# felipefelixarias/a2cat-vn-pytorch

Hardware: NVIDIA B200
Metric: env-steps/s (obs gather+step+reset) (higher is better)
Workload: dtype u8

## Files before the change

a2cat-vn-pytorch_b200/csrc/vn_common.cuh:

```cuda
#pragma once
#include <cuda_runtime.h>
#include <stdint.h>

#include <cstdarg>
#include <cstdio>

#include "vn_b200.h"

#if defined(__CUDA_ARCH__) && (__CUDA_ARCH__ < 1000)
#error "libvn_b200 is written for sm_100a (B200) only"
#endif

namespace vn {

void set_error(const char *fmt, ...);
int32_t launch_result(const char *what, cudaError_t e);
template <typename... P>
inline bool aligned16(const P *...p) {
    return ((reinterpret_cast<uintptr_t>(p) | ... | uintptr_t(0)) & 15) == 0;
}
int sm_count();
int32_t ensure_smem(const void *kernel, int bytes);
template <typename... KArgs>
int32_t ensure_smem(void (*kernel)(KArgs...), int bytes) {
// ... 123 lines not shown
__device__ __forceinline__ uint64_t l2_policy_evict_last() {
    uint64_t p;
    asm volatile("createpolicy.fractional.L2::evict_last.b64 %0, 1.0;" : "=l"(p));
    return p;
}
__device__ __forceinline__ void bulk_g2s_hint(void *smem_dst, const void *gmem_src, uint32_t bytes, uint64_t *bar,
                                              uint64_t policy) {
    asm volatile(
        "cp.async.bulk.shared::cluster.global.mbarrier::complete_tx::bytes.L2::cache_hint [%0], [%1], %2, [%3], %4;" ::"r"(
            smem_u32(smem_dst)),
        "l"(gmem_src), "r"(bytes), "r"(smem_u32(bar)), "l"(policy)
        : "memory");
}
__device__ __forceinline__ void bulk_s2g_hint(void *gmem_dst, const void *smem_src, uint32_t bytes, uint64_t policy) {
    asm volatile("cp.async.bulk.global.shared::cta.bulk_group.L2::cache_hint [%0], [%1], %2, %3;" ::"l"(gmem_dst),
                 "r"(smem_u32(smem_src)), "r"(bytes), "l"(policy)
                 : "memory");
}
__device__ __forceinline__ void bulk_commit() { asm volatile("cp.async.bulk.commit_group;" ::: "memory"); }
template <int N>
__device__ __forceinline__ void bulk_wait_read() {
    asm volatile("cp.async.bulk.wait_group.read %0;" ::"n"(N) : "memory");
}
__device__ __forceinline__ void fence_proxy_async() { asm volatile("fence.proxy.async.shared::cta;" ::: "memory"); }

}
```

a2cat-vn-pytorch_b200/csrc/vn_env.cu:

```cuda
#include <atomic>
#include <chrono>
#include <cstring>
#include <map>
#include <mutex>
#include <string>
#include <utility>

#include "vn_common.cuh"

namespace vn {

static thread_local std::string g_error;
static unsigned long long *g_gather_trace = nullptr;
static std::atomic<long long> g_launches{0};

void set_error(const char *fmt, ...) {
    char buf[512];
    va_list ap;
    va_start(ap, fmt);
    vsnprintf(buf, sizeof(buf), fmt, ap);
    va_end(ap);
    g_error = buf;
}

// ... 209 lines not shown
__device__ __forceinline__ void add_stats(uint64_t *stats, const EnvStats &s) {
    unsigned long long *st = reinterpret_cast<unsigned long long *>(stats);
    if (s.episodes) {
        atomicAdd(st + VN_STAT_EPISODES, (unsigned long long)s.episodes);
        atomicAdd(reinterpret_cast<double *>(st + VN_STAT_RETURN_SUM), (double)s.ret);
        atomicAdd(st + VN_STAT_LENGTH_SUM, (unsigned long long)s.len);
        if (s.succ) atomicAdd(st + VN_STAT_SUCCESSES, (unsigned long long)s.succ);
        if (s.trunc) atomicAdd(st + VN_STAT_TRUNCATIONS, (unsigned long long)s.trunc);
    }
    if (s.coll) atomicAdd(st + VN_STAT_COLLISIONS, (unsigned long long)s.coll);
    if (s.steps) atomicAdd(st + VN_STAT_STEPS, (unsigned long long)s.steps);
    if (s.resets) atomicAdd(st + VN_STAT_RESETS, (unsigned long long)s.resets);
    if (s.skipped) atomicAdd(st + VN_STAT_ROWS_SKIPPED, (unsigned long long)s.skipped);
}

__device__ __forceinline__ void signal_host(const vn_step_out_t &out) {
    __syncthreads();
    if (threadIdx.x == 0) {
        __threadfence_system();
        *reinterpret_cast<volatile uint32_t *>(out.host_seq + blockIdx.x) = out.seq;
    }
}

template <bool kReset>
__global__ void __launch_bounds__(kStepThreads) vn_step_kernel(const StepParams p) {
    const bool defer_wait = (p.out.flags & VN_STEP_ACTIONS_READY) && !(p.out.flags & VN_STEP_NO_OVERLAP) &&
                            p.out.gather_desc != nullptr;
    if (!defer_wait) asm volatile("griddepcontrol.wait;" ::: "memory");
    asm volatile("griddepcontrol.launch_dependents;" ::: "memory");
    const int i = blockIdx.x * blockDim.x + threadIdx.x;
    if (i == 0 && p.out.sched) p.out.sched[p.out.parity & 1] = 0u;
    EnvStats st;
    if (i < p.env.n_envs) {
        int rec, grec;
        step_env<kReset>(p, i, st, rec, grec);
        if (p.out.gather_desc)
            reinterpret_cast<int2 *>(p.out.gather_desc)[(size_t)(p.out.parity & 1) * p.env.n_envs + i] =
                make_int2(rec, grec);
    }

    if (p.out.stats) {
        const EnvStats w = warp_reduce(st);
        if ((threadIdx.x & 31) == 0) add_stats(p.out.stats, w);
    }
    if (p.out.host_seq) signal_host(p.out);
    if (defer_wait) asm volatile("griddepcontrol.wait;" ::: "memory");
}

struct GatherParams {
    vn_store_t store;
    const int2 *desc;
    const int32_t *obs_state;
    const int32_t *goal;
    const uint8_t *did_reset;
    uint8_t *obs[VN_MAX_PLANES];
    uint8_t *goal_obs[VN_MAX_PLANES];
    unsigned int *sched;
    int32_t n;
    int32_t parity;
    int32_t early_release;
    unsigned long long *trace;
};

__device__ __forceinline__ unsigned long long globaltimer_ns() {
    unsigned long long t;
    asm volatile("mov.u64 %0, %globaltimer;" : "=l"(t));
    return t;
}

template <int kThreads, int kUnroll>
__device__ __forceinline__ void copy_segment16(const uint8_t *__restrict__ src, uint8_t *__restrict__ dst, int n16) {
    const int4 *s = reinterpret_cast<const int4 *>(src);
    int4 *d = reinterpret_cast<int4 *>(dst);
    int base = threadIdx.x;
    for (; base + (kUnroll - 1) * kThreads < n16; base += kUnroll * kThreads) {
        int4 v[kUnroll];
#pragma unroll
        for (int k = 0; k < kUnroll; ++k) v[k] = ld_stream16(s + base + k * kThreads);
#pragma unroll
        for (int k = 0; k < kUnroll; ++k) st_stream16(d + base + k * kThreads, v[k]);
    }
    int4 v[kUnroll];
// ... 26 lines not shown
                if (p.obs[pl])
                    copy_segment16<kThreads, kUnroll>(src + p.store.plane_off[pl],
                                                      p.obs[pl] + (size_t)env * p.store.plane_bytes[pl],
                                                      p.store.plane_bytes[pl] >> 4);
            }
        }
        if (grec >= 0) {
            const uint8_t *gsrc = p.store.base + (size_t)grec * p.store.state_pitch;
#pragma unroll 1
            for (int pl = 0; pl < p.store.n_planes; ++pl) {
                if (p.goal_obs[pl])
                    copy_segment16<kThreads, kUnroll>(gsrc + p.store.plane_off[pl],
                                                      p.goal_obs[pl] + (size_t)env * p.store.plane_bytes[pl],
                                                      p.store.plane_bytes[pl] >> 4);
            }
        }
    }
}

struct L2Policies {
    uint64_t load, store;
};

template <typename F>
__device__ __forceinline__ void bulk_copy_slice(const vn_store_t &st, const uint8_t *src, uint8_t *const *dst, int env,
                                                int slice, int split, uint8_t *smem, uint64_t *bar, uint32_t &parity,
                                                const L2Policies &pol, F while_loading, bool whole) {
    bulk_wait_read<0>();
    int total = 0;
#pragma unroll 1
    for (int pl = 0; pl < st.n_planes; ++pl)
        if (dst[pl]) {
            const int n16 = st.plane_bytes[pl] >> 4, per = (n16 + split - 1) / split;
            const int lo = min(slice * per, n16), hi = min(lo + per, n16);
            total += hi - lo;
        }
    if (total == 0) return;
    if (whole && split == 1) {
        int first = -1, last = -1;
        for (int pl = 0; pl < st.n_planes; ++pl)
            if (dst[pl]) {
                if (first < 0) first = pl;
                last = pl;
            }
        const uint32_t base = (uint32_t)st.plane_off[first];
        const uint32_t span = (uint32_t)st.plane_off[last] + (uint32_t)st.plane_bytes[last] - base;
        mbar_expect_tx(bar, span);
        bulk_g2s_hint(smem, src + base, span, bar, pol.load);
        while_loading();
        mbar_wait(bar, parity & 1u);
        parity ^= 1u;
        for (int pl = first; pl <= last; ++pl)
            if (dst[pl])
                bulk_s2g_hint(dst[pl] + (size_t)env * st.plane_bytes[pl], smem + ((uint32_t)st.plane_off[pl] - base),
                              (uint32_t)st.plane_bytes[pl], pol.store);
        bulk_commit();
        return;
    }
    mbar_expect_tx(bar, (uint32_t)total << 4);
    int off = 0;
#pragma unroll 1
    for (int pl = 0; pl < st.n_planes; ++pl)
        if (dst[pl]) {
            const int n16 = st.plane_bytes[pl] >> 4, per = (n16 + split - 1) / split;
            const int lo = min(slice * per, n16), hi = min(lo + per, n16);
            if (hi > lo)
                bulk_g2s_hint(smem + ((size_t)off << 4), src + st.plane_off[pl] + ((size_t)lo << 4),
                              (uint32_t)(hi - lo) << 4, bar, pol.load);
            off += hi - lo;
        }
    while_loading();
    mbar_wait(bar, parity & 1u);
    parity ^= 1u;
    off = 0;
#pragma unroll 1
    for (int pl = 0; pl < st.n_planes; ++pl)
        if (dst[pl]) {
            const int n16 = st.plane_bytes[pl] >> 4, per = (n16 + split - 1) / split;
            const int lo = min(slice * per, n16), hi = min(lo + per, n16);
            if (hi > lo)
                bulk_s2g_hint(dst[pl] + (size_t)env * st.plane_bytes[pl] + ((size_t)lo << 4), smem + ((size_t)off << 4),
                              (uint32_t)(hi - lo) << 4, pol.store);
            off += hi - lo;
        }
    bulk_commit();
}

__global__ void __launch_bounds__(32) vn_gather_bulk_kernel(const GatherParams p, int split, unsigned int *sched,
                                                            int whole) {
    extern __shared__ __align__(128) uint8_t smem[];
    __shared__ uint64_t bar;
    if (threadIdx.x != 0) return;
    unsigned long long *tr = p.trace ? p.trace + (size_t)blockIdx.x * 16 : nullptr;
    if (tr) {
        tr[0] = globaltimer_ns();
        unsigned int smid;
        asm volatile("mov.u32 %0, %smid;" : "=r"(smid));
        tr[6] = smid;
    }
    mbar_init(&bar, 1);
    asm volatile("fence.mbarrier_init.release.cluster;" ::: "memory");
    asm volatile("griddepcontrol.wait;" ::: "memory");
    if (p.early_release) asm volatile("griddepcontrol.launch_dependents;" ::: "memory");
    if (tr) tr[1] = globaltimer_ns();
    int n_units = 0;
    uint32_t parity = 0;
    const L2Policies pol{l2_policy_evict_last(), l2_policy_evict_first()};
    const int units = p.n * split;
    const bool dynamic = sched != nullptr;
    auto unit_desc = [&](int u) -> int2 {
        if (u >= units) return make_int2(-1, -1);
        const int env = split == 1 ? u : u / split;
        if (p.desc) return p.desc[env];
        int2 d = make_int2(p.obs_state[env], -1);
        if (p.goal && (!p.did_reset || p.did_reset[env])) d.y = p.goal[env];
        return d;
    };
    int u = (int)blockIdx.x;
    int2 d = unit_desc(u);
    while (u < units) {
        const int env = split == 1 ? u : u / split;
        const int slice = split == 1 ? 0 : u - env * split;
        int u_next = 0;
        int2 d_next = make_int2(-1, -1);
        bool have_next = false;
        auto fetch_next = [&]() {
            if (have_next) return;
            u_next = dynamic ? (int)gridDim.x + (int)atomicAdd(sched, 1u) : u + (int)gridDim.x;
            d_next = unit_desc(u_next);
            have_next = true;
        };
        if (d.x >= 0) {
            const uint8_t *src = p.store.base + (size_t)d.x * p.store.state_pitch;
            bulk_copy_slice(p.store, src, p.obs, env, slice, split, smem, &bar, parity, pol, fetch_next,
                            (whole & 1) != 0);
        }
        if (d.y >= 0) {
            const uint8_t *gsrc = p.store.base + (size_t)d.y * p.store.state_pitch;
            bulk_copy_slice(p.store, gsrc, p.goal_obs, env, slice, split, smem, &bar, parity, pol, fetch_next,
                            (whole & 2) != 0);
        }
        fetch_next();
        if (tr) {
            if (n_units == 0) tr[2] = globaltimer_ns();
            tr[3] = globaltimer_ns();
            if (n_units < 8) tr[8 + n_units] = tr[3] | ((unsigned long long)(d.x < 0 && d.y < 0) << 63);
            ++n_units;
        }
        u = u_next;
        d = d_next;
    }
    bulk_wait_read<0>();
    if (tr) {
        tr[4] = globaltimer_ns();
        tr[5] = (unsigned long long)n_units;
    }
}

constexpr int kFusedWarps = 4;
constexpr int kFusedPerSm = 4;

template <bool kReset>
__global__ void __launch_bounds__(kFusedWarps * 32) vn_step_fused_kernel(const StepParams sp, const GatherParams gp) {
    extern __shared__ __align__(128) uint8_t smem[];
    __shared__ uint64_t bar[kFusedWarps];
    __shared__ int s_rec, s_grec;
    const int warp = threadIdx.x >> 5;
    if (threadIdx.x < kFusedWarps) mbar_init(&bar[threadIdx.x], 1);
    asm volatile("fence.mbarrier_init.release.cluster;" ::: "memory");
    asm volatile("griddepcontrol.wait;" ::: "memory");
    asm volatile("griddepcontrol.launch_dependents;" ::: "memory");
    const int env = blockIdx.x;
    if (threadIdx.x == 0) {
        EnvStats st;
        int rec, grec;
        step_env<kReset>(sp, env, st, rec, grec);
        if (sp.out.stats) add_stats(sp.out.stats, st);
        if (sp.out.gather_desc)
// ... 186 lines not shown
}

static int32_t check_rows_aligned(const GatherParams &gp) {
    for (int pl = 0; pl < gp.store.n_planes; ++pl) {
        VN_REQUIRE(aligned16(gp.obs[pl]), "gather: obs[%d] must be 16-byte aligned", pl);
        VN_REQUIRE(aligned16(gp.goal_obs[pl]), "gather: goal_obs[%d] must be 16-byte aligned", pl);
    }
    return VN_OK;
}

static int plane_set_bytes(const vn_store_t &st, uint8_t *const *dst, bool use, int *span, bool *contiguous) {
    int sum = 0, first = -1, last = -1;
    for (int pl = 0; pl < st.n_planes; ++pl)
        if (use && dst[pl]) {
            sum += st.plane_bytes[pl];
            if (first < 0) first = pl;
            last = pl;
        }
    *span = first < 0 ? 0 : st.plane_off[last] + st.plane_bytes[last] - st.plane_off[first];
    *contiguous = first >= 0 && last > first && *span - sum <= 128 * (last - first);
    return sum;
}

static int32_t launch_gather(const GatherParams &gp, int32_t variant, cudaStream_t stream) {
    if (gp.n == 0) return VN_OK;
    int32_t rc = check_rows_aligned(gp);
    if (rc) return rc;
    if (variant == VN_GATHER_AUTO || variant == VN_GATHER_FUSED || variant == VN_GATHER_PERSISTENT)
        variant = VN_GATHER_BULK;
    if (variant == VN_GATHER_LDG) {
        constexpr int kThreads = 256;
        return launch(vn_gather_ldg_kernel<kThreads, 4>, "vn_gather_ldg_kernel", dim3(gp.n), dim3(kThreads), 0, stream,
                      true, gp);
    }
    if (variant != VN_GATHER_BULK) {
        set_error("gather: unknown variant %d", variant);
        return VN_EINVAL;
    }
    int split = gp.n < 2 * sm_count() ? min(16, (2 * sm_count() + gp.n - 1) / gp.n) : 1;
    int per_env = 0, per_goal = 0;
    for (int pl = 0; pl < gp.store.n_planes; ++pl) {
        if (gp.obs[pl]) per_env += gp.store.plane_bytes[pl];
        if (gp.goal && gp.goal_obs[pl]) per_goal += gp.store.plane_bytes[pl];
    }
    split = max(split, (max(per_env, per_goal) + 52 * 1024 - 1) / (52 * 1024));
    int smem_obs = 0, smem_goal = 0;
    for (int pl = 0; pl < gp.store.n_planes; ++pl) {
        const int n16 = gp.store.plane_bytes[pl] >> 4, per = (n16 + split - 1) / split;
        if (gp.obs[pl]) smem_obs += per << 4;
        if (gp.goal && gp.goal_obs[pl]) smem_goal += per << 4;
    }
    int smem = max(smem_obs, smem_goal), whole = 0;
    if (split == 1) {
        int span_o, span_g;
        bool co, cg;
        plane_set_bytes(gp.store, gp.obs, true, &span_o, &co);
        plane_set_bytes(gp.store, gp.goal_obs, gp.goal != nullptr, &span_g, &cg);
        if (co) smem = max(smem, span_o);
        if (cg) smem = max(smem, span_g);
        whole = (co ? 1 : 0) | (cg ? 2 : 0);
    }
    VN_REQUIRE(smem <= 200 * 1024, "gather(bulk): %d bytes of planes per env exceed shared memory", smem);
    rc = ensure_smem(vn_gather_bulk_kernel, smem);
    if (rc) return rc;
    const int grid = (int)min((int64_t)gp.n * split, (int64_t)sm_count() * ctas_per_sm(smem));
    return launch(vn_gather_bulk_kernel, "vn_gather_bulk_kernel", dim3(grid), dim3(32), (size_t)smem, stream, true, gp,
                  split, gp.sched ? gp.sched + (gp.parity & 1) : nullptr, whole);
}
// ... 40 lines not shown
                  dim3(kStepThreads), 0, static_cast<cudaStream_t>(stream), true, sp);
}

static int32_t make_gather_params(GatherParams &gp, const vn_store_t *store, const vn_envs_t *envs,
                                  const vn_step_out_t *out, bool *any) {
    int32_t rc = validate_store(store);
    if (rc) return rc;
    VN_REQUIRE(envs->goal, "envs: null pointer");
    VN_REQUIRE(out && out->obs_state, "out: obs_state is required");
    gp.store = *store;
    gp.obs_state = out->obs_state;
    gp.n = envs->n_envs;
    bool any_goal = false, any_obs = false;
    for (int pl = 0; pl < VN_MAX_PLANES; ++pl) {
        gp.obs[pl] = pl < store->n_planes ? out->obs[pl] : nullptr;
        gp.goal_obs[pl] = pl < store->n_planes ? out->goal_obs[pl] : nullptr;
        any_goal |= gp.goal_obs[pl] != nullptr;
        any_obs |= gp.obs[pl] != nullptr;
    }
    gp.goal = any_goal ? envs->goal : nullptr;
    gp.did_reset = out->did_reset;
    gp.sched = out->sched;
    gp.parity = out->parity;
    gp.early_release = 1;
    gp.trace = g_gather_trace;
    gp.desc = out->gather_desc
                  ? reinterpret_cast<const int2 *>(out->gather_desc) + (size_t)(out->parity & 1) * envs->n_envs
                  : nullptr;
    VN_REQUIRE(!any_goal || out->did_reset, "out: did_reset is required when goal planes are emitted");
    *any = any_goal || any_obs;
    return VN_OK;
}

static int32_t run_gather(const vn_store_t *store, const vn_envs_t *envs, const vn_step_out_t *out, int32_t variant,
                          void *stream) {
    VN_REQUIRE(envs && envs->n_envs >= 0, "envs: null or negative n_envs");
    if (envs->n_envs == 0) return VN_OK;
    GatherParams gp;
    bool any = false;
    int32_t rc = make_gather_params(gp, store, envs, out, &any);
    if (rc) return rc;
    if (!any) return VN_OK;
    return launch_gather(gp, variant, static_cast<cudaStream_t>(stream));
}

static int32_t fused_smem_bytes(const vn_store_t *store, const vn_step_out_t *out) {
    bool any_goal = false;
    for (int pl = 0; pl < store->n_planes; ++pl) any_goal |= out->goal_obs[pl] != nullptr;
    const int64_t smem = store->state_pitch * (any_goal ? 2 : 1);
    return smem <= 200 * 1024 ? (int32_t)smem : -1;
}

static int32_t run_fused(const vn_store_t *store, const vn_tables_t *tab, const vn_envs_t *envs, const vn_rules_t *rules,
                         const vn_inject_t *inj, const int32_t *actions, const uint8_t *mask, const vn_step_out_t *out,
                         void *stream, bool reset, int32_t *actions_copy, int32_t smem) {
    StepParams sp;
    int32_t rc = make_step_params(sp, tab, envs, rules, inj, actions, mask, out, reset, actions_copy);
    if (rc) return rc;
    sp.skip_rows = (out->flags & VN_STEP_SKIP_UNCHANGED) != 0;
    GatherParams gp;
    bool any = false;
    rc = make_gather_params(gp, store, envs, out, &any);
    if (!rc) rc = check_rows_aligned(gp);
    if (rc) return rc;
    const auto kernel = reset ? vn_step_fused_kernel<true> : vn_step_fused_kernel<false>;
    rc = ensure_smem(kernel, smem);
// ... 90 lines not shown
                *smem = ps;
                return kModePersistent;
            }
        }
    }
    return kModeSplit;
}

static int32_t run_step(const vn_store_t *store, const vn_tables_t *tab, const vn_envs_t *envs, const vn_rules_t *rules,
                        const vn_inject_t *inj, const int32_t *actions, const uint8_t *mask, const vn_step_out_t *out,
                        int32_t variant, void *stream, bool reset) {
    VN_REQUIRE(envs && envs->n_envs >= 0, "envs: null or negative n_envs");
    if (envs->n_envs == 0) return VN_OK;
    int32_t rc = validate_store(store);
    if (rc) return rc;
    int32_t smem = 0;
    const StepMode mode = choose_mode(store, envs, out, variant, &smem);
    if (mode == kModeError) return VN_EINVAL;
    if (mode == kModeFused)
        rc = run_fused(store, tab, envs, rules, inj, actions, mask, out, stream, reset, nullptr, smem);
    else if (mode == kModePersistent)
        rc = run_persistent(store, tab, envs, rules, inj, actions, mask, out, stream, reset, nullptr, smem);
    else {
        rc = run_scalar(tab, envs, rules, inj, actions, mask, out, stream, reset);
        if (rc) return rc;
        rc = run_gather(store, envs, out, variant, stream);
    }
    if (rc) return rc;
    return run_float_leaves(store, envs, out, stream);
}

static bool is_mapped_host(const void *p) {
    constexpr int kSlots = 8;
    static thread_local const void *known[kSlots] = {nullptr};
    static thread_local int next = 0;
    for (int i = 0; i < kSlots; ++i)
        if (known[i] == p) return true;
    cudaPointerAttributes pa;
    if (cudaPointerGetAttributes(&pa, p) != cudaSuccess) {
        cudaGetLastError();
        return false;
    }
    if (pa.type != cudaMemoryTypeHost || pa.devicePointer == nullptr) return false;
    known[next] = p;
    next = (next + 1) % kSlots;
    return true;
}

}
// ... 64 lines not shown
                      int32_t gather_variant, void *stream) {
    return vn::run_gather(store, envs, out, gather_variant, stream);
}

int32_t vn_env_step_host(const vn_store_t *store, const vn_tables_t *tables, const vn_envs_t *envs,
                         const vn_rules_t *rules, const vn_inject_t *inject, const int32_t *host_actions,
                         int32_t *dev_actions_copy, const vn_step_out_t *out, void *ready_event,
                         int32_t gather_variant, void *stream) {
    VN_REQUIRE(envs && envs->n_envs >= 0, "envs: null or negative n_envs");
    if (envs->n_envs == 0) return VN_OK;
    int32_t rc = vn::validate_store(store);
    if (rc) return rc;
    VN_REQUIRE(host_actions, "step_host: host_actions is null");
    VN_REQUIRE(vn::is_mapped_host(host_actions),
               "step_host: host_actions must be pinned (page-locked, device-mapped) host memory");
    VN_REQUIRE(!out || !out->host_pack || vn::is_mapped_host(out->host_pack),
               "step_host: out->host_pack must be pinned (page-locked, device-mapped) host memory");
    VN_REQUIRE(!out || !out->host_seq || vn::is_mapped_host(out->host_seq),
               "step_host: out->host_seq must be pinned (page-locked, device-mapped) host memory");
    int32_t smem = 0;
    const vn::StepMode mode = vn::choose_mode(store, envs, out, gather_variant, &smem);
    if (mode == vn::kModeError) return VN_EINVAL;
    const bool one_launch = mode != vn::kModeSplit;
    if (mode == vn::kModeFused)
        rc = vn::run_fused(store, tables, envs, rules, inject, host_actions, nullptr, out, stream, false,
                           dev_actions_copy, smem);
    else if (mode == vn::kModePersistent)
        rc = vn::run_persistent(store, tables, envs, rules, inject, host_actions, nullptr, out, stream, false,
                                dev_actions_copy, smem);
    else
        rc = vn::run_scalar(tables, envs, rules, inject, host_actions, nullptr, out, stream, false, dev_actions_copy);
    if (rc) return rc;
    if (ready_event) {
        cudaError_t e = cudaEventRecord(static_cast<cudaEvent_t>(ready_event), static_cast<cudaStream_t>(stream));
        if (e != cudaSuccess) {
            vn::set_error("step_host: event record: %s", cudaGetErrorString(e));
            return VN_ECUDA;
        }
    }
    if (!one_launch) {
        rc = vn::run_gather(store, envs, out, gather_variant, stream);
        if (rc) return rc;
    }
    return vn::run_float_leaves(store, envs, out, stream);
}

int32_t vn_env_step_mode(const vn_store_t *store, const vn_envs_t *envs, const vn_step_out_t *out,
                         int32_t gather_variant) {
    VN_REQUIRE(envs && envs->n_envs >= 0, "envs: null or negative n_envs");
    int32_t rc = vn::validate_store(store);
    if (rc) return rc;
    int32_t smem = 0;
    const vn::StepMode mode = vn::choose_mode(store, envs, out, gather_variant, &smem);
    return mode == vn::kModeError ? VN_EINVAL : (int32_t)mode;
}

int32_t vn_env_host_seq_words(const vn_store_t *store, const vn_envs_t *envs, const vn_step_out_t *out,
                              int32_t gather_variant) {
    VN_REQUIRE(envs && envs->n_envs >= 0, "envs: null or negative n_envs");
    int32_t rc = vn::validate_store(store);
    if (rc) return rc;
    int32_t smem = 0;
    const vn::StepMode mode = vn::choose_mode(store, envs, out, gather_variant, &smem);
    if (mode == vn::kModeError) return VN_EINVAL;
// ... 92 lines not shown
    VN_REQUIRE(event, "event_wait: null");
    cudaError_t e = cudaEventSynchronize(static_cast<cudaEvent_t>(event));
    if (e != cudaSuccess) {
        vn::set_error("event_wait: %s", cudaGetErrorString(e));
        return VN_ECUDA;
    }
    return VN_OK;
}

int32_t vn_gather_plane(const vn_store_t *store, int32_t plane, const int32_t *idx, int32_t n, uint8_t *out,
                        int32_t gather_variant, void *stream) {
    int32_t rc = vn::validate_store(store);
    if (rc) return rc;
    VN_REQUIRE(plane >= 0 && plane < store->n_planes, "gather_plane: plane=%d", plane);
    VN_REQUIRE(idx && out && n >= 0, "gather_plane: null pointer");
    vn::GatherParams gp;
    gp.store = *store;
    gp.obs_state = idx;
    gp.goal = nullptr;
    gp.did_reset = nullptr;
    gp.desc = nullptr;
    gp.sched = nullptr;
    gp.parity = 0;
    gp.early_release = 0;
    gp.trace = nullptr;
    gp.n = n;
    for (int pl = 0; pl < VN_MAX_PLANES; ++pl) {
        gp.obs[pl] = (pl == plane) ? out : nullptr;
        gp.goal_obs[pl] = nullptr;
    }
    return vn::launch_gather(gp, gather_variant, static_cast<cudaStream_t>(stream));
}

}
```

a2cat-vn-pytorch_b200/lib.py:

```python
import ctypes as C
import os

from . import build as _build

VN_MAX_PLANES = 6
VN_N_STATS = 9

RULE_COLLISION_SKIPS_GOAL = 0x01
RULE_NEG_STEP_REWARD = 0x02
RULE_COLLISION_OVERRIDES = 0x04
RULE_TERM_PREV_OBS = 0x08
RULE_TWO_LEVEL = 0x10
RULE_NOOP_ACTION = 0x20
RULE_AUTO_RESET = 0x40

GATHER_AUTO, GATHER_LDG, GATHER_BULK, GATHER_FUSED, GATHER_PERSISTENT = 0, 1, 2, 3, 4
STEP_ACTIONS_READY = 0x01
STEP_SKIP_UNCHANGED = 0x02
STEP_NO_OVERLAP = 0x04
MODE_SPLIT, MODE_FUSED, MODE_PERSISTENT = 0, 1, 2
ABI_VERSION = 4
STAT_NAMES = ("episodes", "return_sum", "length_sum", "successes", "collisions", "steps", "truncations", "resets",
              "rows_skipped")

_P = C.c_void_p


class Store(C.Structure):
    _fields_ = [("base", _P), ("state_pitch", C.c_int64), ("n_states", C.c_int32), ("n_planes", C.c_int32),
                ("plane_off", C.c_int32 * VN_MAX_PLANES), ("plane_bytes", C.c_int32 * VN_MAX_PLANES)]


class Tables(C.Structure):
    _fields_ = [("adj", _P), ("task_goal", _P), ("task_cand_off", _P), ("task_prefix", _P), ("cand_state", _P),
                ("n_states", C.c_int32), ("n_tasks", C.c_int32)]


class Envs(C.Structure):
    _fields_ = [("n_envs", C.c_int32), ("env_id_base", C.c_int32), ("state", _P), ("goal", _P), ("task", _P),
                ("elapsed", _P), ("epoch", _P), ("ep_return", _P), ("ep_length", _P), ("task_lo", _P),
                ("task_cnt", _P)]


class Rules(C.Structure):
    _fields_ = [("reward_goal", C.c_float), ("reward_step", C.c_float), ("reward_collision", C.c_float),
                ("max_episode_steps", C.c_int32), ("goal_compare", C.c_int32), ("flags", C.c_int32),
                ("n_actions", C.c_int32), ("reserved", C.c_int32), ("seed", C.c_uint64)]

# ... 145 lines not shown
```

a2cat-vn-pytorch_b200/vec_env.py:

```python
import ctypes as C
import weakref

import numpy as np
import torch

from . import lib as L
from . import spaces
from .store import DeviceWorld
from .tables import World, Family

try:
    _raw_stream = torch._C._cuda_getCurrentRawStream
except AttributeError:
    def _raw_stream(index):
        return torch.cuda.current_stream(index).cuda_stream

OBS_LAYOUTS = {
    "aux5": ("rgb", "goal_rgb", "depth", "segmentation", "goal_segmentation"),
    "frame": "rgb",
    "pair": ("rgb", "goal_rgb"),
    "dict": {"image": "rgb", "goal": "goal_rgb"},
    "thor6": ("rgb", "depth", "segmentation", "tp_rgb", "tp_depth", "tp_segmentation"),
    "rgbd_goal": ("rgb", "goal_rgb", "depth"),
}
# ... 99 lines not shown
                 episode_info=True, skip_unchanged=True, numpy_obs=False):
        self.dw = device_world if device_world is not None else DeviceWorld(world, device)
        self.world: World = self.dw.world
        self.family: Family = self.world.family
        self.lib = self.dw.lib
        self.device = self.dw.device
        self.rank, self.world_size = rank, world_size
        self.num_envs_total = num_envs
        lo, hi = shard_range(num_envs, rank, world_size)
        self.env_lo, self.num_envs = lo, hi - lo
        n = self.num_envs
        self.max_episode_steps = int(max_episode_steps or 0)
        self.obs_layout = obs_layout
        self.unreal_wrapper = unreal_wrapper
        self.host_outputs = host_outputs
        self.scaled_float = scaled_float
        self.numpy_obs = numpy_obs
        self._host_stage = {}
        self.episode_info = episode_info
        self.n_actions = 4
        self.gather = {"auto": L.GATHER_AUTO, "ldg": L.GATHER_LDG, "bulk": L.GATHER_BULK,
                       "fused": L.GATHER_FUSED, "persistent": L.GATHER_PERSISTENT}[gather]
        self._step_flags = L.STEP_SKIP_UNCHANGED if skip_unchanged else 0
        lay = self.world.layout
        self.leaves = resolve_layout(obs_layout)
        names = self.leaves.values() if isinstance(self.leaves, dict) else \
            (self.leaves if isinstance(self.leaves, tuple) else (self.leaves,))
        self.obs_planes = tuple(dict.fromkeys(x for x in names if not x.startswith("goal_")))
        self.goal_planes = tuple(dict.fromkeys(x[5:] for x in names if x.startswith("goal_")))
        for p in self.obs_planes + self.goal_planes:
            if p not in lay.planes:
                raise ValueError("obs_layout %r needs plane %r in the store (has %s)" % (obs_layout, p, lay.planes))

        tasks = self._default_env_tasks(num_envs) if env_tasks is None else np.asarray(env_tasks, np.int32)
        if tasks.shape != (num_envs, 2):
            raise ValueError("env_tasks must be [num_envs, 2] (lo, count)")
        if (tasks[:, 1] < 1).any() or (tasks[:, 0] < 0).any() or (tasks.sum(1) > len(self.world.tasks)).any():
            raise ValueError("env_tasks ranges fall outside the task table")
        tasks = tasks[lo:hi]

        h, w = lay.frame_hw
        with torch.cuda.device(self.device):
            i32 = lambda: torch.zeros(n, dtype=torch.int32, device=self.device)
            self.state, self.goal, self.task, self.elapsed, self.ep_length = i32(), i32(), i32(), i32(), i32()
            self.epoch = i32()
            self.ep_return = torch.zeros(n, dtype=torch.float32, device=self.device)
            self.task_lo = torch.from_numpy(np.ascontiguousarray(tasks[:, 0])).to(self.device)
            self.task_cnt = torch.from_numpy(np.ascontiguousarray(tasks[:, 1])).to(self.device)
            self._pack = torch.zeros(n * 20, dtype=torch.uint8, device=self.device)
            self.reward = self._pack[:4 * n].view(torch.float32)
            self.episode_return = self._pack[4 * n:8 * n].view(torch.float32)
            self.episode_length = self._pack[8 * n:12 * n].view(torch.int32)
            self.info_state = self._pack[12 * n:16 * n].view(torch.int32)
            self.done = self._pack[16 * n:17 * n]
            self.truncated = self._pack[17 * n:18 * n]
            self.win = self._pack[18 * n:19 * n]
            self.did_reset = self._pack[19 * n:20 * n]
            self.lar = torch.zeros((n, self.n_actions + 1), dtype=torch.float32, device=self.device)
            self.obs_state = i32()
            self.stats = torch.zeros(L.VN_N_STATS, dtype=torch.int64, device=self.device)
            self.actions_dev = i32()
            self._sched = torch.zeros(4, dtype=torch.int32, device=self.device)
            self._gather_desc = torch.zeros((2, max(n, 1), 2), dtype=torch.int32, device=self.device)
            if scaled_float:
                self.obs_buf, self.goal_buf = {}, {}
                chw = lambda p: (n, lay.channels[lay.planes.index(p)], h, w)
                self.float_buf = {("goal_" + p if g else p): torch.zeros(chw(p), dtype=torch.float32, device=self.device)
                                  for g, ps in ((False, self.obs_planes), (True, self.goal_planes)) for p in ps}
            else:
                self.obs_buf = {p: lay.batch(p, n, self.device) for p in self.obs_planes}
                self.goal_buf = {p: lay.batch(p, n, self.device) for p in self.goal_planes}
                self.float_buf = {}
            self._pack_hosts = [torch.zeros(n * 20, dtype=torch.uint8).pin_memory() for _ in range(2)]
            self._pack_host = self._pack_hosts[0]
            self._actions_host = torch.zeros(n, dtype=torch.int32).pin_memory()
        self._inject_keep = None
        self._c_inject = None
        if inject is not None:
            self.set_inject(*inject)

        self._c_envs = L.Envs(n, lo, *(t.data_ptr() for t in (self.state, self.goal, self.task, self.elapsed,
                                                              self.epoch, self.ep_return, self.ep_length,
                                                              self.task_lo, self.task_cnt)))
        fam = self.family
        flags = 0
# ... 173 lines not shown
        r = self._ref
        self._call(self.lib.vn_env_reset, r["store"], r["tables"], r["envs"], r["rules"],
                   C.byref(self._c_inject) if self._c_inject is not None else None,
                   L.ptr(m), r["out"], self.gather, self._stream())
        if self.scaled_float:
            self._convert_float_leaves()
        return self._obs_out()

    def _mode_of(self, out, flags):
        key = (id(out), bool(flags & L.STEP_ACTIONS_READY))
        m = self._modes.get(key)
        if m is None:
            saved = out.flags
            out.flags = flags
            m = self.lib.vn_env_step_mode(C.byref(self.dw.store), C.byref(self._c_envs), C.byref(out), self.gather)
            out.flags = saved
            if m < 0:
                L.check(m)
            self._modes[key] = m
        return m

    def _tick(self, out, flags):
        self._calls += 1
        out.parity = self._calls & 1
        if flags & L.STEP_ACTIONS_READY and (self._serial_next or self._prev_mode != L.MODE_SPLIT):
            flags |= L.STEP_NO_OVERLAP
        self._serial_next = False
        out.flags = flags
        self._prev_mode = self._mode_of(out, flags)

    def step_async(self, actions, actions_ready=False):
        self._check_open()
        if self._pending:
            raise RuntimeError("step_async() called again before step_wait()")
        inj = C.byref(self._c_inject) if self._c_inject is not None else None
        if self.host_outputs and not (torch.is_tensor(actions) and actions.is_cuda):
            a = np.asarray(actions.cpu() if torch.is_tensor(actions) else actions).reshape(-1)
            if a.size != self.num_envs:
                raise ValueError("expected %d actions, got %d" % (self.num_envs, a.size))
            self._actions_np[:] = a
            self._last_actions = self._actions_np
            self._tick(self._c_out_host, L.STEP_ACTIONS_READY | self._step_flags)
            self._seq = (self._seq % 0x7FFFFFFF) + 1
            self._c_out_host.seq = self._seq
            self._next_pack()
            r = self._ref
            self._call(self.lib.vn_env_step_host, r["store"], r["tables"], r["envs"], r["rules"], inj,
                       self._actions_host.data_ptr(), self.actions_dev.data_ptr(), r["out_host"], None,
                       self.gather, self._stream())
# ... 117 lines not shown
        hc = L.HostCall()
        hc.store = C.cast(C.pointer(self.dw.store), C.c_void_p)
        hc.tables = C.cast(C.pointer(self.dw.tables), C.c_void_p)
        hc.envs = C.cast(C.pointer(self._c_envs), C.c_void_p)
        hc.rules = C.cast(C.pointer(self._c_rules), C.c_void_p)
        hc.inject = C.cast(C.pointer(self._c_inject), C.c_void_p) if self._c_inject is not None else None
        hc.host_actions, hc.dev_actions_copy = self._actions_ptr, self._actions_dev_ptr
        hc.out = C.cast(C.pointer(self._c_out_host), C.c_void_p)
        hc.seq_words, hc.gather_variant, hc.timeout_us = self._seq_words, self.gather, 60_000_000
        self._hc, self._hc_ptr = hc, C.addressof(hc)
        self._hc_inject = self._c_inject
        self._hc_fn = self.lib.vn_env_step_host_call

    def step(self, actions):
        if self.host_outputs and type(actions) is np.ndarray and not self._pending and not self.closed \
                and actions.size == self.num_envs and self.num_envs and \
                (not self.scaled_float or self._float_leaves is not None):
            n = self.num_envs
            np.copyto(self._actions_np, actions if actions.ndim == 1 else actions.reshape(-1), casting="same_kind")
            if self._hc is None or self._hc_inject is not self._c_inject:
                self._bind_host_call()
            out = self._c_out_host
            self._calls += 1
            out.parity = self._calls & 1
            if self._serial_next or self._prev_mode != L.MODE_SPLIT:
                out.flags = L.STEP_ACTIONS_READY | L.STEP_NO_OVERLAP | self._step_flags
                self._serial_next = False
                self._prev_mode = self._mode_of(out, out.flags)
            else:
                out.flags = L.STEP_ACTIONS_READY | self._step_flags
            self._seq = out.seq = (self._seq % 0x7FFFFFFF) + 1
            self._next_pack()
            res = np.empty(5 * n, np.uint8)
            ptr = res.__array_interface__["data"][0]
            if torch.cuda.current_device() == self._dev_index:
                rc = self._hc_fn(self._hc_ptr, ptr, ptr + 4 * n, _raw_stream(self._dev_index))
            else:
                with torch.cuda.device(self.device):
                    rc = self._hc_fn(self._hc_ptr, ptr, ptr + 4 * n, _raw_stream(self._dev_index))
            if rc:
                L.check(rc)
            noop = (self._actions_np < 0) if self.family.noop_action else None
            infos = LazyInfos(self, self._pack_np, noop, True)
            self._infos_refs[self._slot] = weakref.ref(infos)
            return self._obs_out(), res[:4 * n].view(np.float32), res[4 * n:].view(np.bool_), infos
        self.step_async(actions)
        return self.step_wait()

    def close(self):
        if not self.closed and torch.cuda.is_available():
            torch.cuda.synchronize(self.device)
        self.closed = True

# ... 42 lines not shown
            self._opt = (torch.from_numpy(act).to(self.device), torch.from_numpy(dst).to(self.device))
        act, dst = self._opt
        t, s = self.task.long(), self.state.long()
        return act[t, s], dst[t, s]

    def state_dict(self):
        keys = ("state", "goal", "task", "elapsed", "epoch", "ep_return", "ep_length", "stats")
        d = {k: getattr(self, k).cpu().clone() for k in keys}
        d["complexity"] = self.dw.complexity
        return d

    def load_state_dict(self, d):
        for k in ("state", "goal", "task", "elapsed", "epoch", "ep_return", "ep_length", "stats"):
            getattr(self, k).copy_(d[k].to(self.device))
        self.set_complexity(d.get("complexity"))
        self.gather_current()

    def gather_current(self):
        for p, buf in self.obs_buf.items():
            gather_plane(self.dw, p, self.state, out=buf, variant=self.gather)
        for p, buf in self.goal_buf.items():
            gather_plane(self.dw, p, self.goal, out=buf, variant=self.gather)
        self.obs_state.copy_(self.state)
        if self.scaled_float:
            self._convert_float_leaves(all_rows=True)
        return self._obs()


def gather_plane(dw: DeviceWorld, plane, idx, out=None, variant=L.GATHER_AUTO):
    pi = dw.plane_index(plane)
    lay = dw.world.layout
    h, w = lay.frame_hw
    idx = idx.to(device=dw.device, dtype=torch.int32).contiguous()
    n = idx.numel()
    if out is None:
        out = lay.batch(plane, n, dw.device)
    elif n > 1 and out.stride(0) != lay.plane_bytes[pi]:
        raise ValueError("gather_plane: rows of `out` must be %d bytes apart (StoreLayout.batch)" % lay.plane_bytes[pi])
    with torch.cuda.device(dw.device):
        L.check(dw.lib.vn_gather_plane(C.byref(dw.store), pi, idx.data_ptr(), n, out.data_ptr(), variant,
                                       torch.cuda.current_stream(dw.device).cuda_stream))
    return out


def reduce_stats(vec, device=None, group=None):
    import torch.distributed as dist
# ... 9 lines not shown
```

include/vn_b200.h:

```cpp
#ifndef VN_B200_H
#define VN_B200_H

#include <stdint.h>

#ifdef __cplusplus
extern "C" {
#endif

#define VN_ABI_VERSION 4
#define VN_MAX_PLANES 6

#define VN_OK 0
#define VN_EINVAL (-1)
#define VN_ECUDA (-2)
#define VN_EUNSUPPORTED (-3)

#define VN_RULE_COLLISION_SKIPS_GOAL 0x01
#define VN_RULE_NEG_STEP_REWARD 0x02
#define VN_RULE_COLLISION_OVERRIDES 0x04
#define VN_RULE_TERM_PREV_OBS 0x08
#define VN_RULE_TWO_LEVEL 0x10
#define VN_RULE_NOOP_ACTION 0x20
#define VN_RULE_AUTO_RESET 0x40

#define VN_STEP_ACTIONS_READY 0x01
#define VN_STEP_NO_OVERLAP 0x04
#define VN_STEP_SKIP_UNCHANGED 0x02

#define VN_GOAL_FULL 0
#define VN_GOAL_POSITION 1
#define VN_GOAL_NEVER 2

#define VN_STAT_EPISODES 0
#define VN_STAT_RETURN_SUM 1
#define VN_STAT_LENGTH_SUM 2
#define VN_STAT_SUCCESSES 3
#define VN_STAT_COLLISIONS 4
#define VN_STAT_STEPS 5
#define VN_STAT_TRUNCATIONS 6
#define VN_STAT_RESETS 7
#define VN_STAT_ROWS_SKIPPED 8
#define VN_N_STATS 9

typedef struct vn_store {
    const uint8_t *base;
    int64_t state_pitch;
    int32_t n_states;
    int32_t n_planes;
    int32_t plane_off[VN_MAX_PLANES];
// ... 62 lines not shown
    int32_t *episode_length;
    int32_t *info_state;
    int32_t *obs_state;
    uint64_t *stats;
    int32_t *gather_desc;
    int32_t parity;
    int32_t flags;
    uint32_t *sched;
    uint8_t *host_pack;
    uint32_t *host_seq;
    uint32_t seq;
    uint32_t reserved;
    int32_t *rec_action;
    float *rec_reward;
    uint8_t *rec_done;
    int32_t *rec_state;
    int32_t *rec_goal;
    const vn_float_leaf_t *float_leaves;
    int32_t n_float_leaves;
    int32_t float_h, float_w;
    int32_t reserved2;
} vn_step_out_t;

#define VN_GATHER_AUTO 0
#define VN_GATHER_LDG 1
#define VN_GATHER_BULK 2
#define VN_GATHER_FUSED 3
#define VN_GATHER_PERSISTENT 4

int32_t vn_abi_version(void);
int32_t vn_abi_struct_size(int32_t which);
const char *vn_last_error(void);
int64_t vn_launch_count(void);

int32_t vn_fill_store(const vn_store_t *store, int32_t record0, int32_t n_records, uint64_t seed, int32_t scene,
                      int32_t state0, const int32_t *plane_ids , void *stream);

int32_t vn_env_reset(const vn_store_t *store, const vn_tables_t *tables, const vn_envs_t *envs,
                     const vn_rules_t *rules, const vn_inject_t *inject, const uint8_t *mask,
                     const vn_step_out_t *out, int32_t gather_variant, void *stream);

int32_t vn_env_step(const vn_store_t *store, const vn_tables_t *tables, const vn_envs_t *envs,
                    const vn_rules_t *rules, const vn_inject_t *inject, const int32_t *actions,
                    const vn_step_out_t *out, int32_t gather_variant, void *stream);

int32_t vn_env_step_scalar(const vn_tables_t *tables, const vn_envs_t *envs, const vn_rules_t *rules,
// ... 129 lines not shown
```

Measured before the change: 123.8 million.

## Overlap bulk gather with step kernel via per-row and per-block release/acquire flags

Adds fine-grained flag words in the sched buffer so the gather kernel can start before the step kernel finishes. The gather waits per step block for its descriptors and per env row for the previous consumer, publishing each row once its bulk stores complete. This replaces the whole-grid griddepcontrol.wait barrier with spin-waits on release/acquire flags, aiming to hide step/gather serialization. It adds spin and fence overhead and a risk of deadlock or ordering bugs. Parity now carries a monotonically increasing step counter.

```diff
diff --git a/a2cat-vn-pytorch_b200/csrc/vn_common.cuh b/a2cat-vn-pytorch_b200/csrc/vn_common.cuh
--- a/a2cat-vn-pytorch_b200/csrc/vn_common.cuh
+++ b/a2cat-vn-pytorch_b200/csrc/vn_common.cuh
@@ -169,6 +169,20 @@
 __device__ __forceinline__ void bulk_wait_read() {
     asm volatile("cp.async.bulk.wait_group.read %0;" ::"n"(N) : "memory");
 }
+template <int N>
+__device__ __forceinline__ void bulk_wait() {
+    asm volatile("cp.async.bulk.wait_group %0;" ::"n"(N) : "memory");
+}
 __device__ __forceinline__ void fence_proxy_async() { asm volatile("fence.proxy.async.shared::cta;" ::: "memory"); }
+__device__ __forceinline__ void fence_proxy_async_global() { asm volatile("fence.proxy.async.global;" ::: "memory"); }
+
+__device__ __forceinline__ uint32_t ld_acquire_gpu(const uint32_t *p) {
+    uint32_t v;
+    asm volatile("ld.acquire.gpu.global.u32 %0, [%1];" : "=r"(v) : "l"(p) : "memory");
+    return v;
+}
+__device__ __forceinline__ void st_release_gpu(uint32_t *p, uint32_t v) {
+    asm volatile("st.release.gpu.global.u32 [%0], %1;" ::"l"(p), "r"(v) : "memory");
+}
 
 }
diff --git a/a2cat-vn-pytorch_b200/csrc/vn_env.cu b/a2cat-vn-pytorch_b200/csrc/vn_env.cu
--- a/a2cat-vn-pytorch_b200/csrc/vn_env.cu
+++ b/a2cat-vn-pytorch_b200/csrc/vn_env.cu
@@ -255,6 +255,8 @@
     }
 }
 
+__device__ __forceinline__ uint32_t *step_words(uint32_t *sched, int n) { return sched + 8 + n; }
+
 template <bool kReset>
 __global__ void __launch_bounds__(kStepThreads) vn_step_kernel(const StepParams p) {
     const bool defer_wait = (p.out.flags & VN_STEP_ACTIONS_READY) && !(p.out.flags & VN_STEP_NO_OVERLAP) &&
@@ -262,14 +264,23 @@
     if (!defer_wait) asm volatile("griddepcontrol.wait;" ::: "memory");
     asm volatile("griddepcontrol.launch_dependents;" ::: "memory");
     const int i = blockIdx.x * blockDim.x + threadIdx.x;
-    if (i == 0 && p.out.sched) p.out.sched[p.out.parity & 1] = 0u;
+    const int slot = p.out.parity & 1;
+    const uint32_t step = (uint32_t)p.out.parity;
+    const int blocks = (int)gridDim.x;
+    uint32_t *const words = p.out.sched ? step_words(p.out.sched, p.env.n_envs) : nullptr;
+    if (defer_wait && words) {
+        if (threadIdx.x == 0)
+            while (ld_acquire_gpu(words + blocks + blockIdx.x) != step - 1u) {
+            }
+        __syncthreads();
+    }
+    if (i == 0 && p.out.sched) p.out.sched[slot] = 0u;
     EnvStats st;
     if (i < p.env.n_envs) {
         int rec, grec;
         step_env<kReset>(p, i, st, rec, grec);
         if (p.out.gather_desc)
-            reinterpret_cast<int2 *>(p.out.gather_desc)[(size_t)(p.out.parity & 1) * p.env.n_envs + i] =
-                make_int2(rec, grec);
+            reinterpret_cast<int2 *>(p.out.gather_desc)[(size_t)slot * p.env.n_envs + i] = make_int2(rec, grec);
     }
 
     if (p.out.stats) {
@@ -277,7 +288,18 @@
         if ((threadIdx.x & 31) == 0) add_stats(p.out.stats, w);
     }
     if (p.out.host_seq) signal_host(p.out);
+    if (words) {
+        __syncthreads();
+        if (threadIdx.x == 0) {
+            __threadfence();
+            st_release_gpu(words + blockIdx.x, step);
+        }
+    }
     if (defer_wait) asm volatile("griddepcontrol.wait;" ::: "memory");
+    if (words && threadIdx.x == 0) {
+        __threadfence();
+        st_release_gpu(words + blocks + blockIdx.x, step);
+    }
 }
 
 struct GatherParams {
@@ -291,6 +313,7 @@
     unsigned int *sched;
     int32_t n;
     int32_t parity;
+    int32_t rows;
     int32_t early_release;
     unsigned long long *trace;
 };
@@ -363,10 +386,14 @@
     uint64_t load, store;
 };
 
-template <typename F>
+struct NoHook {
+    __device__ __forceinline__ void operator()() const {}
+};
+template <typename F, typename B = NoHook>
 __device__ __forceinline__ void bulk_copy_slice(const vn_store_t &st, const uint8_t *src, uint8_t *const *dst, int env,
                                                 int slice, int split, uint8_t *smem, uint64_t *bar, uint32_t &parity,
-                                                const L2Policies &pol, F while_loading, bool whole) {
+                                                const L2Policies &pol, F while_loading, bool whole,
+                                                B before_store = B()) {
     bulk_wait_read<0>();
     int total = 0;
 #pragma unroll 1
@@ -391,6 +418,7 @@
         while_loading();
         mbar_wait(bar, parity & 1u);
         parity ^= 1u;
+        before_store();
         for (int pl = first; pl <= last; ++pl)
             if (dst[pl])
                 bulk_s2g_hint(dst[pl] + (size_t)env * st.plane_bytes[pl], smem + ((uint32_t)st.plane_off[pl] - base),
@@ -413,6 +441,7 @@
     while_loading();
     mbar_wait(bar, parity & 1u);
     parity ^= 1u;
+    before_store();
     off = 0;
 #pragma unroll 1
     for (int pl = 0; pl < st.n_planes; ++pl)
@@ -441,9 +470,37 @@
     }
     mbar_init(&bar, 1);
     asm volatile("fence.mbarrier_init.release.cluster;" ::: "memory");
-    asm volatile("griddepcontrol.wait;" ::: "memory");
+    const bool overlap = p.rows == 2;
+    if (!overlap) asm volatile("griddepcontrol.wait;" ::: "memory");
     if (p.early_release) asm volatile("griddepcontrol.launch_dependents;" ::: "memory");
     if (tr) tr[1] = globaltimer_ns();
+    uint32_t *const rows = p.rows ? p.sched + 8 : nullptr;
+    const uint32_t *const ready = overlap ? step_words(p.sched, p.n) : nullptr;
+    const uint32_t step = (uint32_t)p.parity;
+    uint32_t spins = 0;
+    int ready_block = -1;
+    auto acquire_ready = [&](int block) {
+        if (block == ready_block) return;
+        while ((int32_t)(ld_acquire_gpu(ready + block) - step) < 0) ++spins;
+        ready_block = block;
+    };
+    bool tickets_ready = !overlap;
+    int old_row = -1, new_row = -1;
+    auto publish_old = [&]() {
+        if (old_row < 0) return;
+        bulk_wait<1>();
+        fence_proxy_async_global();
+        st_release_gpu(rows + old_row, step);
+        old_row = -1;
+    };
+    bool acquired = false;
+    auto acquire_row = [&](int env) {
+        if (acquired) return;
+        acquired = true;
+        if (!overlap) return;
+        while (ld_acquire_gpu(rows + env) != step - 1u) ++spins;
+        fence_proxy_async_global();
+    };
     int n_units = 0;
     uint32_t parity = 0;
     const L2Policies pol{l2_policy_evict_last(), l2_policy_evict_first()};
@@ -452,7 +509,10 @@
     auto unit_desc = [&](int u) -> int2 {
         if (u >= units) return make_int2(-1, -1);
         const int env = split == 1 ? u : u / split;
-        if (p.desc) return p.desc[env];
+        if (p.desc) {
+            if (overlap) acquire_ready(env / kStepThreads);
+            return p.desc[env];
+        }
         int2 d = make_int2(p.obs_state[env], -1);
         if (p.goal && (!p.did_reset || p.did_reset[env])) d.y = p.goal[env];
         return d;
@@ -467,21 +527,43 @@
         bool have_next = false;
         auto fetch_next = [&]() {
             if (have_next) return;
+            if (dynamic && !tickets_ready) {
+                acquire_ready(0);
+                tickets_ready = true;
+            }
             u_next = dynamic ? (int)gridDim.x + (int)atomicAdd(sched, 1u) : u + (int)gridDim.x;
             d_next = unit_desc(u_next);
             have_next = true;
         };
+        auto while_loading = [&]() {
+            fetch_next();
+            if (rows) publish_old();
+        };
+        auto before_store = [&]() {
+            if (rows) acquire_row(env);
+        };
+        acquired = false;
         if (d.x >= 0) {
             const uint8_t *src = p.store.base + (size_t)d.x * p.store.state_pitch;
-            bulk_copy_slice(p.store, src, p.obs, env, slice, split, smem, &bar, parity, pol, fetch_next,
-                            (whole & 1) != 0);
+            bulk_copy_slice(p.store, src, p.obs, env, slice, split, smem, &bar, parity, pol, while_loading,
+                            (whole & 1) != 0, before_store);
         }
         if (d.y >= 0) {
             const uint8_t *gsrc = p.store.base + (size_t)d.y * p.store.state_pitch;
-            bulk_copy_slice(p.store, gsrc, p.goal_obs, env, slice, split, smem, &bar, parity, pol, fetch_next,
-                            (whole & 2) != 0);
+            bulk_copy_slice(p.store, gsrc, p.goal_obs, env, slice, split, smem, &bar, parity, pol, while_loading,
+                            (whole & 2) != 0, before_store);
         }
         fetch_next();
+        if (rows) {
+            acquire_row(env);
+            if (d.x >= 0 || d.y >= 0) {
+                publish_old();
+                old_row = new_row;
+                new_row = env;
+            } else {
+                st_release_gpu(rows + env, step);
+            }
+        }
         if (tr) {
             if (n_units == 0) tr[2] = globaltimer_ns();
             tr[3] = globaltimer_ns();
@@ -491,10 +573,18 @@
         u = u_next;
         d = d_next;
     }
-    bulk_wait_read<0>();
+    if (rows) {
+        bulk_wait<0>();
+        fence_proxy_async_global();
+        if (old_row >= 0) st_release_gpu(rows + old_row, step);
+        if (new_row >= 0) st_release_gpu(rows + new_row, step);
+    } else {
+        bulk_wait_read<0>();
+    }
     if (tr) {
         tr[4] = globaltimer_ns();
         tr[5] = (unsigned long long)n_units;
+        tr[7] = spins;
     }
 }
 
@@ -727,7 +817,17 @@
     return sum;
 }
 
-static int32_t launch_gather(const GatherParams &gp, int32_t variant, cudaStream_t stream) {
+static int bulk_split(const GatherParams &gp) {
+    const int split = gp.n < 2 * sm_count() ? min(16, (2 * sm_count() + gp.n - 1) / gp.n) : 1;
+    int per_env = 0, per_goal = 0;
+    for (int pl = 0; pl < gp.store.n_planes; ++pl) {
+        if (gp.obs[pl]) per_env += gp.store.plane_bytes[pl];
+        if (gp.goal && gp.goal_obs[pl]) per_goal += gp.store.plane_bytes[pl];
+    }
+    return max(split, (max(per_env, per_goal) + 52 * 1024 - 1) / (52 * 1024));
+}
+
+static int32_t launch_gather(GatherParams gp, int32_t variant, cudaStream_t stream) {
     if (gp.n == 0) return VN_OK;
     int32_t rc = check_rows_aligned(gp);
     if (rc) return rc;
@@ -742,13 +842,8 @@
         set_error("gather: unknown variant %d", variant);
         return VN_EINVAL;
     }
-    int split = gp.n < 2 * sm_count() ? min(16, (2 * sm_count() + gp.n - 1) / gp.n) : 1;
-    int per_env = 0, per_goal = 0;
-    for (int pl = 0; pl < gp.store.n_planes; ++pl) {
-        if (gp.obs[pl]) per_env += gp.store.plane_bytes[pl];
-        if (gp.goal && gp.goal_obs[pl]) per_goal += gp.store.plane_bytes[pl];
-    }
-    split = max(split, (max(per_env, per_goal) + 52 * 1024 - 1) / (52 * 1024));
+    const int split = bulk_split(gp);
+    gp.rows = gp.sched && split == 1 ? (gp.rows == 2 ? 2 : 1) : 0;
     int smem_obs = 0, smem_goal = 0;
     for (int pl = 0; pl < gp.store.n_planes; ++pl) {
         const int n16 = gp.store.plane_bytes[pl] >> 4, per = (n16 + split - 1) / split;
@@ -835,6 +930,7 @@
     gp.did_reset = out->did_reset;
     gp.sched = out->sched;
     gp.parity = out->parity;
+    gp.rows = 0;
     gp.early_release = 1;
     gp.trace = g_gather_trace;
     gp.desc = out->gather_desc
@@ -846,7 +942,7 @@
 }
 
 static int32_t run_gather(const vn_store_t *store, const vn_envs_t *envs, const vn_step_out_t *out, int32_t variant,
-                          void *stream) {
+                          void *stream, bool overlap = false) {
     VN_REQUIRE(envs && envs->n_envs >= 0, "envs: null or negative n_envs");
     if (envs->n_envs == 0) return VN_OK;
     GatherParams gp;
@@ -854,7 +950,19 @@
     int32_t rc = make_gather_params(gp, store, envs, out, &any);
     if (rc) return rc;
     if (!any) return VN_OK;
+    gp.rows = overlap ? 2 : 0;
     return launch_gather(gp, variant, static_cast<cudaStream_t>(stream));
+}
+
+static bool gather_overlaps(const vn_store_t *store, const vn_envs_t *envs, const vn_step_out_t *out, int32_t variant) {
+    const int32_t f = out ? out->flags : 0;
+    if (!(f & VN_STEP_OVERLAP_GATHER) || !(f & VN_STEP_ACTIONS_READY) || (f & VN_STEP_NO_OVERLAP)) return false;
+    if (variant == VN_GATHER_LDG || !out->gather_desc || !out->sched || (out->float_leaves && out->n_float_leaves > 0))
+        return false;
+    GatherParams gp;
+    bool any = false;
+    if (make_gather_params(gp, store, envs, out, &any) != VN_OK) return false;
+    return any && bulk_split(gp) == 1;
 }
 
 static int32_t fused_smem_bytes(const vn_store_t *store, const vn_step_out_t *out) {
@@ -991,9 +1099,10 @@
     else if (mode == kModePersistent)
         rc = run_persistent(store, tab, envs, rules, inj, actions, mask, out, stream, reset, nullptr, smem);
     else {
+        const bool overlap = gather_overlaps(store, envs, out, variant);
         rc = run_scalar(tab, envs, rules, inj, actions, mask, out, stream, reset);
         if (rc) return rc;
-        rc = run_gather(store, envs, out, variant, stream);
+        rc = run_gather(store, envs, out, variant, stream, overlap);
     }
     if (rc) return rc;
     return run_float_leaves(store, envs, out, stream);
@@ -1104,6 +1213,7 @@
     const vn::StepMode mode = vn::choose_mode(store, envs, out, gather_variant, &smem);
     if (mode == vn::kModeError) return VN_EINVAL;
     const bool one_launch = mode != vn::kModeSplit;
+    const bool overlap = !one_launch && vn::gather_overlaps(store, envs, out, gather_variant);
     if (mode == vn::kModeFused)
         rc = vn::run_fused(store, tables, envs, rules, inject, host_actions, nullptr, out, stream, false,
                            dev_actions_copy, smem);
@@ -1121,7 +1231,7 @@
         }
     }
     if (!one_launch) {
-        rc = vn::run_gather(store, envs, out, gather_variant, stream);
+        rc = vn::run_gather(store, envs, out, gather_variant, stream, overlap);
         if (rc) return rc;
     }
     return vn::run_float_leaves(store, envs, out, stream);
@@ -1260,6 +1370,7 @@
     gp.desc = nullptr;
     gp.sched = nullptr;
     gp.parity = 0;
+    gp.rows = 0;
     gp.early_release = 0;
     gp.trace = nullptr;
     gp.n = n;
diff --git a/a2cat-vn-pytorch_b200/lib.py b/a2cat-vn-pytorch_b200/lib.py
--- a/a2cat-vn-pytorch_b200/lib.py
+++ b/a2cat-vn-pytorch_b200/lib.py
@@ -18,12 +18,17 @@
 STEP_ACTIONS_READY = 0x01
 STEP_SKIP_UNCHANGED = 0x02
 STEP_NO_OVERLAP = 0x04
+STEP_OVERLAP_GATHER = 0x08
 MODE_SPLIT, MODE_FUSED, MODE_PERSISTENT = 0, 1, 2
-ABI_VERSION = 4
+ABI_VERSION = 5
 STAT_NAMES = ("episodes", "return_sum", "length_sum", "successes", "collisions", "steps", "truncations", "resets",
               "rows_skipped")
 
 _P = C.c_void_p
+
+
+def sched_words(n_envs):
+    return 8 + n_envs + 2 * ((n_envs + 127) // 128)
 
 
 class Store(C.Structure):
diff --git a/a2cat-vn-pytorch_b200/vec_env.py b/a2cat-vn-pytorch_b200/vec_env.py
--- a/a2cat-vn-pytorch_b200/vec_env.py
+++ b/a2cat-vn-pytorch_b200/vec_env.py
@@ -145,6 +145,7 @@
         self.gather = {"auto": L.GATHER_AUTO, "ldg": L.GATHER_LDG, "bulk": L.GATHER_BULK,
                        "fused": L.GATHER_FUSED, "persistent": L.GATHER_PERSISTENT}[gather]
         self._step_flags = L.STEP_SKIP_UNCHANGED if skip_unchanged else 0
+        self._overlap_flag = 0 if self.gather == L.GATHER_LDG or scaled_float else L.STEP_OVERLAP_GATHER
         lay = self.world.layout
         self.leaves = resolve_layout(obs_layout)
         names = self.leaves.values() if isinstance(self.leaves, dict) else \
@@ -183,7 +184,7 @@
             self.obs_state = i32()
             self.stats = torch.zeros(L.VN_N_STATS, dtype=torch.int64, device=self.device)
             self.actions_dev = i32()
-            self._sched = torch.zeros(4, dtype=torch.int32, device=self.device)
+            self._sched = torch.zeros(L.sched_words(n), dtype=torch.int32, device=self.device)
             self._gather_desc = torch.zeros((2, max(n, 1), 2), dtype=torch.int32, device=self.device)
             if scaled_float:
                 self.obs_buf, self.goal_buf = {}, {}
@@ -403,9 +404,12 @@
 
     def _tick(self, out, flags):
         self._calls += 1
-        out.parity = self._calls & 1
-        if flags & L.STEP_ACTIONS_READY and (self._serial_next or self._prev_mode != L.MODE_SPLIT):
-            flags |= L.STEP_NO_OVERLAP
+        out.parity = self._calls
+        if flags & L.STEP_ACTIONS_READY:
+            if self._serial_next or self._prev_mode != L.MODE_SPLIT:
+                flags |= L.STEP_NO_OVERLAP
+            else:
+                flags |= self._overlap_flag
         self._serial_next = False
         out.flags = flags
         self._prev_mode = self._mode_of(out, flags)
@@ -569,13 +573,13 @@
                 self._bind_host_call()
             out = self._c_out_host
             self._calls += 1
-            out.parity = self._calls & 1
+            out.parity = self._calls
             if self._serial_next or self._prev_mode != L.MODE_SPLIT:
                 out.flags = L.STEP_ACTIONS_READY | L.STEP_NO_OVERLAP | self._step_flags
                 self._serial_next = False
                 self._prev_mode = self._mode_of(out, out.flags)
             else:
-                out.flags = L.STEP_ACTIONS_READY | self._step_flags
+                out.flags = L.STEP_ACTIONS_READY | self._overlap_flag | self._step_flags
             self._seq = out.seq = (self._seq % 0x7FFFFFFF) + 1
             self._next_pack()
             res = np.empty(5 * n, np.uint8)
@@ -664,6 +668,7 @@
         for p, buf in self.goal_buf.items():
             gather_plane(self.dw, p, self.goal, out=buf, variant=self.gather)
         self.obs_state.copy_(self.state)
+        self._serial_next = True
         if self.scaled_float:
             self._convert_float_leaves(all_rows=True)
         return self._obs()
diff --git a/include/vn_b200.h b/include/vn_b200.h
--- a/include/vn_b200.h
+++ b/include/vn_b200.h
@@ -7,7 +7,7 @@
 extern "C" {
 #endif
 
-#define VN_ABI_VERSION 4
+#define VN_ABI_VERSION 5
 #define VN_MAX_PLANES 6
 
 #define VN_OK 0
@@ -25,6 +25,7 @@
 
 #define VN_STEP_ACTIONS_READY 0x01
 #define VN_STEP_NO_OVERLAP 0x04
+#define VN_STEP_OVERLAP_GATHER 0x08
 #define VN_STEP_SKIP_UNCHANGED 0x02
 
 #define VN_GOAL_FULL 0
@@ -133,6 +134,8 @@
     int32_t reserved2;
 } vn_step_out_t;
 
+#define VN_SCHED_WORDS(n) (8 + (n) + 2 * (((n) + 127) / 128))
+
 #define VN_GATHER_AUTO 0
 #define VN_GATHER_LDG 1
 #define VN_GATHER_BULK 2
```

After: 130.0 million (median of 6 runs). +5.0%, better.
